# ExcitingSystems/exciting-environments

Measured on AMD Instinct MI355X. Metric: env-steps/sec + achieved HBM GB/s, PMSM Euler fp32 batch=2^22, 1/2/4/8 GPU, higher is better.
Workload: dtype f32

## Files before the change

### exciting-environments_amd/csrc/excenv_api.hip

```cpp
#include <algorithm>
#include <cstdarg>
#include <cstdio>
#include <dlfcn.h>
#include "launch.hpp"

static_assert(EXCENV_FAULT == 0, "EXCENV_FAULT builds exist for tools/isa_guards_selftest.sh only (single objects, never linked into the library)");

namespace excenv {

static thread_local char g_err[512] = "";
thread_local const char* g_last_launch = "";

void set_error(const char* fmt, ...) {
  va_list ap;
  va_start(ap, fmt);
  vsnprintf(g_err, sizeof(g_err), fmt, ap);
  va_end(ap);
}

int launch_transpose(int dtype, int64_t M, int64_t N, const void* in, void* out, hipStream_t stream);
int launch_param_sum(int dtype, int64_t B, int n, const void* const* per_env, void* out, void* workspace, hipStream_t stream);

EnvVTable vtable_pendulum();
EnvVTable vtable_msd();
// ... 6 lines not shown
static const EnvVTable* table(int env) {
  static const EnvVTable T[EXCENV_NUM_ENVS + 1] = {vtable_pendulum(), vtable_msd(),  vtable_cartpole(), vtable_acrobot(),
                                                   vtable_tank(),     vtable_pmsm(), vtable_pmsm_sat()};
  if (env < 0 || env > EXCENV_NUM_ENVS) return nullptr;
  return &T[env];
}

static const EnvVTable* table_public(int env) { return (env >= 0 && env < EXCENV_NUM_ENVS) ? table(env) : nullptr; }

static const EnvVTable* table_for(int env, const excenv_props_t* props, int* rc) {
  *rc = EXCENV_OK;
  if (env < 0 || env >= EXCENV_NUM_ENVS) return nullptr;
  if (props && props->pmsm_lut) {
    const excenv_pmsm_lut_t* l = props->pmsm_lut;
    if (env != EXCENV_PMSM) { set_error("pmsm_lut is only valid for EXCENV_PMSM"); *rc = EXCENV_EINVAL; return nullptr; }
    if (l->n_d < 2 || l->n_q < 2 || !l->grid_d || !l->grid_q || !l->tables) {
      set_error("pmsm_lut: need n_d, n_q >= 2 and non-NULL grid / table pointers");
      *rc = EXCENV_EINVAL;
      return nullptr;
    }
    return table(EXCENV_NUM_ENVS);
  }
  return table(env);
}

static const excenv_launch_opts_t kDefaultOpts = {0, 0, 0, 0};

static int check_opts(const char* fn, const excenv_launch_opts_t*& o) {
  if (!o) o = &kDefaultOpts;
  const int v = o->envs_per_lane;
  if (!(v == 0 || v == 1 || v == 2 || v == 4)) { set_error("%s: opts.envs_per_lane must be 0, 1, 2 or 4 (got %d)", fn, v); return EXCENV_EINVAL; }
  if (o->env_major_mode < 0 || o->env_major_mode > 3) { set_error("%s: opts.env_major_mode must be 0, 1, 2 or 3", fn); return EXCENV_EINVAL; }
  if (o->lds_pad_bytes < 0 || o->lds_pad_bytes > 150 * 1024) { set_error("%s: opts.lds_pad_bytes out of range", fn); return EXCENV_EINVAL; }
  if ((o->flags & ~(EXCENV_OPT_NO_FUSED_ACTIONS | EXCENV_OPT_KEEP_CONSTANT_COLUMNS)) != 0) { set_error("%s: opts.flags has unknown bits set (0x%x)", fn, (unsigned)o->flags); return EXCENV_EINVAL; }
  return EXCENV_OK;
}

static int check_common(const char* fn, int env, int solver, int dtype, int64_t B) {
  if (env < 0 || env >= EXCENV_NUM_ENVS) { set_error("%s: bad env id %d", fn, env); return EXCENV_EINVAL; }
  if (solver < 0 || solver >= EXCENV_NUM_SOLVERS) { set_error("%s: bad solver id %d", fn, solver); return EXCENV_EINVAL; }
  if (dtype != EXCENV_F32 && dtype != EXCENV_F64) { set_error("%s: bad dtype id %d", fn, dtype); return EXCENV_EINVAL; }
  if (B < 0 || B > ((int64_t)1 << 31) * BLOCK) { set_error("%s: bad batch size %lld", fn, (long long)B); return EXCENV_EINVAL; }
  return EXCENV_OK;
}

static int check_control(const char* fn, int env, const excenv_control_t*& c) {
  if (c && c->n_control == 0) c = nullptr;
  if (!c) return EXCENV_OK;
  if (c->n_control < 0 || c->n_control > EXCENV_MAX_CONTROL) { set_error("%s: bad n_control %d", fn, c->n_control); return EXCENV_EINVAL; }
  for (int j = 0; j < c->n_control; ++j) {
    if (c->control_idx[j] < 0 || c->control_idx[j] >= table_public(env)->S) { set_error("%s: control_idx[%d] out of range", fn, j); return EXCENV_EINVAL; }
    if (!c->reference[j]) { set_error("%s: reference[%d] is NULL", fn, j); return EXCENV_ENULL; }
  }
  return EXCENV_OK;
}

}

using namespace excenv;

extern "C" {

int excenv_abi_version(void) { return EXCENV_ABI_VERSION; }

const char* excenv_last_error(void) { return g_err; }

const char* excenv_last_launch(void) { return g_last_launch; }
// ... 689 lines not shown
```

### exciting-environments_amd/csrc/kernels.hpp

```cpp
#pragma once
#include "rk.hpp"
#include "sim_clock.hpp"
#include "sim_plan.hpp"

namespace excenv {

#ifndef EXCENV_FAULT
#define EXCENV_FAULT 0
#endif
template <typename T, class M> struct KProps {
  static constexpr int N = M::P + 2 * M::S + 2 * M::A;
  T scalar[N];
  const T* ptr[N];
  const T* lut_gd;
  const T* lut_gq;
  const T* lut_tab;
  int32_t lut_nd, lut_nq;
  int32_t lut_lds;
};

template <typename T, class M> struct StepArgs {
  KProps<T, M> kp;
  int64_t B;
  const T* state_in[M::S];
// ... 359 lines not shown
      gym_outputs<M, T>(st[0], ob, c, ka.n_control, ka.control_idx, rref, ka.reward + i, ka.terminated + i,
                        ka.truncated + i * tw, 1);
    }
  }
}

template <typename T, int V> constexpr bool aem_shape_ok() { return V * (int)sizeof(T) == 16; }
#define EXCENV_INLINE_ASM_M0_PUSH _Pragma("clang diagnostic push") _Pragma("clang diagnostic ignored \"-Winline-asm\"")
#if EXCENV_FAULT & 4
#define EXCENV_LDS_DIRECT_LOAD(SRC, M0V) EXCENV_INLINE_ASM_M0_PUSH                                                               \
  asm volatile("s_mov_b32 m0, %1\n\tglobal_load_lds_dwordx4 %0, off" ::"v"(SRC), "s"(M0V) : "memory", "m0");                 \
  _Pragma("clang diagnostic pop")
#else
#define EXCENV_LDS_DIRECT_LOAD(SRC, M0V) EXCENV_INLINE_ASM_M0_PUSH                                                               \
  asm volatile("s_mov_b32 m0, %1\n\ts_nop 0\n\tglobal_load_lds_dwordx4 %0, off" ::"v"(SRC), "s"(M0V) : "memory", "m0");      \
  _Pragma("clang diagnostic pop")
#endif
constexpr int AEM_BLOCK_BYTES = 1024 + 16;
template <class M> constexpr int aem_np() { return M::ID == EXCENV_ACROBOT ? 2 : 4; }
template <class M, typename T, int V> constexpr size_t aem_lds_bytes() { return (size_t)(BLOCK / 64) * V * aem_np<M>() * AEM_BLOCK_BYTES; }

template <class M, typename T, bool GENERAL, bool AEM, bool LGYM, int STATES, int SOLVER = -1, bool PLAIN_AHEAD = false, int V = 0> constexpr int sim_min_waves() {
  if (LGYM && (M::ID == EXCENV_ACROBOT || M::ID == EXCENV_CART_POLE) && sizeof(T) == 4 && SOLVER == EXCENV_EULER) return 3;
  if (LGYM && M::ID == EXCENV_ACROBOT && sizeof(T) == 4) return 2;
  if (GENERAL && M::ID == EXCENV_PENDULUM && sizeof(T) == 8) return 2;
  if (AEM && M::IS_PMSM && !M::HAS_LUT && sizeof(T) == 8 && STATES == 0) return 2;
  if (V == 2 && PLAIN_AHEAD && !GENERAL && !AEM && !LGYM && M::IS_PMSM && !M::HAS_LUT && sizeof(T) == 8 && STATES == 0 && SOLVER == EXCENV_EULER) return 2;
  return 1;
}
#define EXCENV_SIM_KERNEL_ATTR __attribute__((amdgpu_waves_per_eu(sim_min_waves<M, T, GENERAL, AEM, LGYM, STATES, SOLVER, AHEAD, V>())))
template <class M, typename T, int SOLVER, bool AHEAD, bool GENERAL, int V, int STATES, bool LUT_LDS = false, bool AEM = false, bool LGYM = false,
          int NT = BLOCK>
__global__ void __launch_bounds__(NT) EXCENV_SIM_KERNEL_ATTR sim_ahead_kernel(const SimArgs<T, M> ka) {
  constexpr bool ACC_T = false;
  [[maybe_unused]] constexpr T acc_step = T(0), acc_end = T(0);
#include "sim_ahead_body.inc"
}
template <class M, typename T, int SOLVER, bool GENERAL, int V, int STATES, bool LUT_LDS = false, int NT = BLOCK>
__global__ void __launch_bounds__(NT) __attribute__((amdgpu_waves_per_eu(sim_min_waves<M, T, GENERAL, false, false, STATES, SOLVER>())))
sim_ahead_acc_t_kernel(const SimArgs<T, M> ka, const T acc_step, const T acc_end) {
  constexpr bool AHEAD = true, AEM = false, LGYM = false, ACC_T = true;
#include "sim_ahead_body.inc"
}

template <typename T, class M> struct ControlFillArgs {
  KProps<T, M> kp;
  int64_t B, rows;
  int32_t n_control, tiled;
  int32_t control_idx[EXCENV_MAX_CONTROL];
  const T* reference[EXCENV_MAX_CONTROL];
  T* obs;
  int64_t o_sk, o_sc, tile_pitch;
};

template <class M, typename T, int V> __global__ void __launch_bounds__(BLOCK) control_fill_kernel(const ControlFillArgs<T, M> ka) {
  const int64_t b0 = ((int64_t)blockIdx.x * BLOCK + threadIdx.x) * V;
  if (b0 >= ka.B) return;
  T* base = ka.obs + (ka.tiled ? (b0 / EXCENV_TILE) * ka.tile_pitch + (b0 % EXCENV_TILE) : b0);
#pragma unroll
  for (int j = 0; j < EXCENV_MAX_CONTROL; ++j) {
    if (j < ka.n_control) {
      const int f = ka.control_idx[j];
      const T lo = ka.kp.scalar[M::P + f], hi = ka.kp.scalar[M::P + M::S + f];
      T r[V], c[V];
      load_v<T, V>(ka.reference[j] + b0, r);
#pragma unroll
      for (int v = 0; v < V; ++v) c[v] = normalize(r[v], lo, hi);
      T* col = base + (M::O + j) * ka.o_sc;
      for (int64_t n = blockIdx.y; n < ka.rows; n += gridDim.y) store_stream<T, V>(col + n * ka.o_sk, c);
    }
  }
}

template <typename T, class M> struct TrajGymArgs {
// ... 147 lines not shown
```

### exciting-environments_amd/csrc/launch.hpp

```cpp
#pragma once
#include <cstdint>
#include <cstdio>
#include <cstring>
#include <type_traits>
#include "kernels_emr.hpp"
#include "refgen.hpp"
#include "rew_vjp.hpp"
#include "step_jac.hpp"
#include "step_vjp.hpp"
#include "vjp.hpp"

namespace excenv {

void set_error(const char* fmt, ...);
static thread_local bool g_attr_failed = false;
extern thread_local const char* g_last_launch;

struct StepCall {
  int vec_pref;
  int solver, dtype;
  int64_t B;
  const excenv_props_t* props;
  const excenv_control_t* control;
  double tau;
// ... 273 lines not shown
  const bool general = batched || ka.n_control > 0 || ka.reward != nullptr;
  int V = 1;
  if (!general) {
    bool ok = true;
    for (int j = 0; j < M::S; ++j) ok &= aligned16(ka.state_in[j]) && aligned16(ka.state_out[j]);
    int want = sc.vec_pref > 0 ? sc.vec_pref : 1;
    if (want > VMAX) want = VMAX;
    while (want > 1 && (sc.B % want) != 0) want >>= 1;
    if (ok) V = want;
  }
  const int64_t lanes = sc.B / V;
  const dim3 grid((unsigned)((lanes + BLOCK - 1) / BLOCK)), block(BLOCK);
  constexpr int VWs = 16 / (int)sizeof(T);
  const bool dense = !general && V == 1 && (M::O % VWs) == 0 && (M::O / VWs) > 1;
  const size_t step_lds = lut_lds_bytes<T, M>(ka.kp, 0, dense ? sizeof(T) * BLOCK * M::O : 0);
  with_solver(sc.solver, [&](auto solver) {
    constexpr int SOLVER = decltype(solver)::value;
    if (general) launch_dyn(&step_kernel<M, T, SOLVER, true, 1>, grid, block, step_lds, sc.stream, ka);
    else with_const<1, 2, 4>(V, [&](auto v) {
      constexpr int VV = decltype(v)::value;
      if constexpr (VV <= VMAX) launch_dyn(&step_kernel<M, T, SOLVER, false, VV>, grid, block, step_lds, sc.stream, ka);
      return true;
    });
    return true;
  });
  g_last_launch = general ? "step_kernel (general)" : V == 1 ? "step_kernel (V=1)" : V == 2 ? "step_kernel (V=2)" : "step_kernel (V=4)";
  return check_launch("excenv_step");
}

template <class M, typename T, int SOLVER, int SEM>
static bool launch_lane_major(const SimPlan& p, SimArgs<T, M> ka, size_t lds_pad, T acc_step, T acc_end, hipStream_t stream) {
  constexpr bool ACC_T = SEM == EXCENV_SEM_AHEAD_ACCUMULATED_T;
  const size_t lds = lut_lds_bytes<T, M>(ka.kp, lds_pad);
  return with_const<SIM_GENERAL, SIM_LEAN, SIM_LEAN_GYM, SIM_AEM>(p.form, [&](auto form) {
    return with_const<1, 2, 4>(p.V, [&](auto v) {
      return with_const<BLOCK, WIDE_THREADS>(p.threads, [&](auto nt) {
        constexpr SimForm F = (SimForm)decltype(form)::value;
        constexpr int V = decltype(v)::value, NT = decltype(nt)::value;
        constexpr bool GEN = F == SIM_GENERAL;
        if constexpr (!sim_instantiated(SimPlan{F, false, V, NT, 0, 0, false, 0, ACC_T}, SEM, M::ID, M::A, (int)sizeof(T), SOLVER,
                                        M::HAS_LUT)) {
          return false;
        } else {
          const dim3 grid((unsigned)((ka.B / V + NT - 1) / NT)), block(NT);
          const size_t l = F == SIM_AEM ? aem_lds_bytes<M, T, V>() + lds : lds;
          with_flag(GEN ? ka.truncated != nullptr : ka.straj[0] != nullptr, [&](auto st) {
            return with_flag(ka.kp.lut_lds != 0, [&](auto lut_lds) {
              constexpr int STATES = (GEN ? -2 : 0) + decltype(st)::value;
              constexpr bool LUT_LDS = M::HAS_LUT && decltype(lut_lds)::value;
              if constexpr (ACC_T)
                launch_dyn(&sim_ahead_acc_t_kernel<M, T, SOLVER, GEN, V, STATES, LUT_LDS, NT>, grid, block, l, stream, ka, acc_step, acc_end);
              else
                launch_dyn(&sim_ahead_kernel<M, T, SOLVER, SEM == EXCENV_SEM_AHEAD, GEN, V, STATES, LUT_LDS, F == SIM_AEM, F == SIM_LEAN_GYM, NT>,
                           grid, block, l, stream, ka);
              return true;
            });
          });
          return true;
        }
      });
    });
  });
}

template <class M, typename T, int SOLVER, int SEM>
static bool launch_em(const SimPlan& p, const SimArgs<T, M>& ka, hipStream_t stream) {
// ... 107 lines not shown
  const bool emr = p.form == SIM_EMR, env_major = emr || p.form == SIM_EM || p.form == SIM_EM_GENERAL;
  if (emr) ka.a_wg = p.period;
  if (!env_major) {
    ka.row_sync = p.row_sync;
    ka.keep_const = (sc.keep_const && sc.traj_layout == EXCENV_LAYOUT_LANE_MAJOR && ka.o_sb == 1 && ka.s_sb == 1) ? 1 : 0;
    const int64_t wg_envs = (int64_t)p.threads * p.V;
    auto wg_off = [&](int layout, int64_t sb, int64_t per_tile) -> int64_t {
      if (layout == EXCENV_LAYOUT_TILED) return (wg_envs == TILE) ? per_tile : -1;
      return wg_envs * sb;
    };
    ka.a_wg = wg_off(sc.action_layout, ka.a_sb, sc.K * M::A * TILE);
    ka.o_wg = wg_off(sc.traj_layout, ka.o_sb, (N + 1) * OW * TILE);
    ka.s_wg = wg_off(sc.traj_layout, ka.s_sb, (N + 1) * TILE);
    if (ka.a_wg < 0 || ka.o_wg < 0 || ka.s_wg < 0) {
      set_error("excenv_sim_ahead: tiled layout needs unbatched properties, no gym trajectories, 16-byte aligned buffers and the %d-byte dtype (control columns are filled by a second launch)", 4);
      return EXCENV_EUNSUPPORTED;
    }
  }
  const size_t lds_pad = (size_t)sc.lds_pad + p.row_lds;
  const T acc_step = (T)(sc.obs_stepsize * (double)sc.substeps), acc_end = (T)((sc.obs_stepsize * (double)sc.substeps) * (double)sc.K);
  auto launch = [&](auto solver, auto sem) {
    constexpr int SOLVER = decltype(solver)::value, SEM = decltype(sem)::value;
    if (emr) return launch_emr<M, T, SOLVER, SEM>(p, ka, sc.stream);
    if (env_major) return launch_em<M, T, SOLVER, SEM>(p, ka, sc.stream);
    return launch_lane_major<M, T, SOLVER, SEM>(p, ka, lds_pad, acc_step, acc_end, sc.stream);
  };
  if (!sim_instantiated(p, sc.semantics, M::ID, M::A, (int)sizeof(T), sc.solver, M::HAS_LUT) || !with_solver(sc.solver, [&](auto solver) {
        return with_const<EXCENV_SEM_STEP, EXCENV_SEM_AHEAD, EXCENV_SEM_AHEAD_ACCUMULATED_T>(sc.semantics, [&](auto sem) { return launch(solver, sem); });
      })) {
    set_error("excenv_sim_ahead: no kernel instantiation for plan '%s' (semantics %d, %d-byte elements)", plan_name(p), sc.semantics,
              (int)sizeof(T));
    return EXCENV_EINVAL;
  }
  g_last_launch = plan_name(p);
  if (int rc = check_launch(emr ? "excenv_sim_ahead (env-major fused, register ring)" : env_major ? "excenv_sim_ahead (env-major fused)" : "excenv_sim_ahead"))
    return rc;
  if (p.split_control) {
    ControlFillArgs<T, M> fa;
    std::memset(&fa, 0, sizeof(fa));
    fa.kp = ka.kp;
    fa.B = sc.B;
    fa.rows = N + 1;
    fa.n_control = ka.n_control;
    fa.tiled = tiled_t ? 1 : 0;
    for (int j = 0; j < ka.n_control; ++j) {
      fa.control_idx[j] = ka.control_idx[j];
      fa.reference[j] = ka.reference[j];
    }
    fa.obs = ka.obs;
    fa.o_sk = ka.o_sk;
    fa.o_sc = ka.o_sc;
    fa.tile_pitch = (N + 1) * OW * TILE;
    bool v4 = (sizeof(T) == 4) && (sc.B % 4 == 0) && aligned16(ka.obs);
    for (int j = 0; j < ka.n_control; ++j) v4 &= aligned16(fa.reference[j]);
    const int64_t lanes = v4 ? sc.B / 4 : sc.B;
    const dim3 fgrid((unsigned)((lanes + BLOCK - 1) / BLOCK), (unsigned)((N + 1 < 64) ? N + 1 : 64)), fblock(BLOCK);
    if (v4) {
      if constexpr (sizeof(T) == 4) hipLaunchKernelGGL((control_fill_kernel<M, T, 4>), fgrid, fblock, 0, sc.stream, fa);
    } else {
      hipLaunchKernelGGL((control_fill_kernel<M, T, 1>), fgrid, fblock, 0, sc.stream, fa);
    }
    return check_launch("excenv_sim_ahead (control columns)");
  }
  return EXCENV_OK;
}

template <class M, typename T> static int launch_traj_gym(const TrajGymCall& gc) {
// ... 151 lines not shown
```

### exciting-environments_amd/csrc/sim_ahead_body.inc

```
  static_assert(!ACC_T || (AHEAD && !AEM && !LGYM), "accumulated time: AHEAD structure, no row-major action windows, no lean gym outputs");
  constexpr int S = M::S, A = M::A, O = M::O;
  extern __shared__ __align__(16) unsigned char excenv_smem[];
  static_assert(NT == BLOCK || (!GENERAL && !AEM && !M::HAS_LUT), "wide workgroups: lean instantiations only (plain or with gym outputs)");
  constexpr bool ROW_BARRIER = NT > BLOCK;
  static_assert(!(GENERAL && V > 1), "per-environment property sets: one environment per lane");
  static_assert(GENERAL == (STATES < 0), "STATES -1 / -2 (general, with / without the gym outputs' code) and 0 / 1 (lean)");
  static_assert(!LGYM || (!GENERAL && !M::HAS_LUT && aem_shape_ok<T, V>()), "lean gym outputs: widest lean form, no look-up model");
  constexpr int NC = GENERAL ? V : 1;
  constexpr bool GYM = GENERAL && STATES == -1;
  static_assert(!AEM || (!GENERAL && !M::HAS_LUT && aem_shape_ok<T, V>() && (16 / (int)sizeof(T)) % A == 0),
                "row-major actions are fused into the widest lean instantiation only");
  const int64_t blk0 = (int64_t)blockIdx.x * (NT * V);
  const unsigned lane_env = threadIdx.x * V;
  const int64_t i0 = blk0 + lane_env;
  Ctx<T, M> cs[NC];
#pragma unroll
  for (int v = 0; v < NC; ++v) {
    load_ctx<GENERAL>(cs[v], ka.kp, (i0 + v < ka.B) ? i0 + v : 0, ka.dt, ka.env_tau, ka.adv_coef);
    cs[v].lin_stop = ka.lin_stop;
    cs[v].lin_div = T(ka.K - 1);
    cs[v].lin_last = ka.K - 1;
  }
  Ctx<T, M>& c = cs[0];
#define EXCENV_CX(v) cs[GENERAL ? (v) : 0]
  stage_lut<M, T>(c, ka.kp);
  if constexpr (M::HAS_LUT) c.lut_lds = LUT_LDS ? 1 : 0;
  if (i0 >= ka.B) return;

  T st[V][S];
#pragma unroll
  for (int j = 0; j < S; ++j) {
    T tmp[V];
    load_v<T, V>(ka.state_in[j] + blk0 + lane_env, tmp);
// ... 125 lines not shown
  constexpr int KC_OBS = 2, KC_LEAF = 6;
  bool keep = false;
  if constexpr (KEEPC) {
    if (__builtin_expect(ka.keep_const != 0, 1)) {
      T kept_o[V], kept_s[V];
      load_v<T, V>(o_blk + KC_OBS * ka.o_sc + o_lane, kept_o);
      if (with_states) load_v<T, V>(ka.straj[KC_LEAF] + s_blk + s_lane, kept_s);
      bool same = true;
#pragma unroll
      for (int v = 0; v < V; ++v) {
        T sv0[S], ob0[O];
#pragma unroll
        for (int j = 0; j < S; ++j) sv0[j] = st[v][j];
        if constexpr (AHEAD) M::post(sv0, c);
        M::observe(sv0, c, ob0);
        same = same & same_bits(kept_o[v], ob0[KC_OBS]);
        if (with_states) same = same & same_bits(kept_s[v], sv0[KC_LEAF]);
      }
      keep = __builtin_amdgcn_readfirstlane((int)(__builtin_amdgcn_ballot_w64(!same) == 0)) != 0;
      if constexpr (V == 1 && !ROW_BARRIER) {
        if (ka.row_sync == 2) {
          unsigned* vote = reinterpret_cast<unsigned*>(excenv_smem);
          if (threadIdx.x == 0) *vote = 0u;
          __syncthreads();
          if (!keep && (threadIdx.x & 63u) == 0u) *vote = 1u;
          __syncthreads();
          keep = __builtin_amdgcn_readfirstlane(*vote) == 0u;
          __syncthreads();
        }
      }
    }
  }

  auto save_row = [&](int64_t n, T (&sv)[V][S]) {
#pragma unroll
    for (int v = 0; v < V; ++v) {
#pragma unroll
      for (int j = 0; j < S; ++j) sv[v][j] = st[v][j];
      if constexpr (AHEAD) {
        if constexpr (M::HAS_LUT) M::post_q(sv[v], c, memo[v]);
        else M::post(sv[v], EXCENV_CX(v));
        if constexpr (M::IS_PMSM) {
          if (deadtime_on) {
            sv[v][0] = aux[v].prev_clip[0];
            sv[v][1] = aux[v].prev_clip[1];
          } else {
            sv[v][0] = T(0);
            sv[v][1] = T(0);
          }
        }
      }
    }
    T ob[V][O];
#pragma unroll
    for (int v = 0; v < V; ++v) M::observe(sv[v], EXCENV_CX(v), ob[v]);
    T* orow = o_blk + n * ka.o_sk;
    bool direct = true;
    if constexpr (ROW_BARRIER) {
      __builtin_amdgcn_s_barrier();
    } else if constexpr (V == 1 && !M::HAS_LUT && !AEM) {
      if (ka.row_sync == 2) {
        constexpr int VE = 16 / (int)sizeof(T), CH = NT / (64 * VE), NW = NT / 64;
        const int OWr = O + (GENERAL ? ka.n_control : 0);
        const int NS = OWr + (with_states ? S : 0);
        T* buf = reinterpret_cast<T*>(excenv_smem) + (unsigned)(n & 1) * (unsigned)(NS * NT);
#pragma unroll
// ... 120 lines not shown
      }
      if (n > 0) {
        store_stream<T, V>(ka.reward + (n - 1) * ka.g_sk + e0, rew);
        store_flags<V>(ka.terminated + (n - 1) * ka.g_sk + e0, fl);
      }
    }
    if constexpr (LGYM && M::IS_PMSM) {
      T rew[V];
      uint8_t fl[V];
#pragma unroll
      for (int v = 0; v < V; ++v) {
        rew[v] = pmsm_reward<M, T>(sv[v], c, has_id, g_id[v], has_iq, g_iq[v], has_tq, g_tq[v]);
        const T nd = normalize(sv[v][3], c.smin[3], c.smax[3]), nq = normalize(sv[v][4], c.smin[4], c.smax[4]);
        fl[v] = sqrt_exceeds_one(nd * nd + nq * nq);
      }
      const int64_t e0 = blk0 + lane_env;
      store_flags<V>(ka.truncated + n * ka.t_sk + e0, fl);
      if (n > 0) {
        store_stream<T, V>(ka.reward + (n - 1) * ka.g_sk + e0, rew);
        store_flags<V>(ka.terminated + (n - 1) * ka.g_sk + e0, fl);
      }
    }
    if constexpr (GYM) {
      if (ka.truncated != nullptr) {
        const int64_t e = i0;
        uint8_t* tr = ka.truncated + e * ka.t_sb + n * ka.t_sk;
        const bool tail = n > 0;
        T* rw = tail ? ka.reward + e * ka.g_sb + (n - 1) * ka.g_sk : nullptr;
        uint8_t* te = tail ? ka.terminated + e * ka.g_sb + (n - 1) * ka.g_sk : nullptr;
        gym_outputs<M, T>(sv[0], ob[0], c, ka.n_control, ka.control_idx, rref[0], rw, te, tr, ka.t_sc);
      }
    }
  };
  auto publish_last = [&](const T (&sv)[V][S]) {
#pragma unroll
    for (int j = 0; j < S; ++j) {
      T tmp[V];
#pragma unroll
      for (int v = 0; v < V; ++v) tmp[v] = sv[v][j];
      store_v<T, V>(ka.last_state[j] + blk0 + lane_env, tmp);
    }
  };
  T sv[V][S];
  if (N == 0) {
    save_row(0, sv);
    publish_last(sv);
    return;
  }

  T a0[A][V], a1[A][V];
  int64_t k = 0, kn = 0;
  int32_t sub = 0, subn = 0;
  constexpr int VW = 16 / (int)sizeof(T);
  constexpr int SP = AEM ? VW / A : 1;
  constexpr int NP = aem_np<M>();
  constexpr int EPI = 64 / NP;
  static_assert(64 % NP == 0, "a load instruction covers whole windows");
  const unsigned wave = threadIdx.x / 64u, lane64 = threadIdx.x % 64u;
  const unsigned wave_off = AEM ? __builtin_amdgcn_readfirstlane(wave * (unsigned)(V * NP * AEM_BLOCK_BYTES)) : 0u;
  const unsigned wave_lds = (unsigned)(uintptr_t)(__attribute__((address_space(3))) unsigned char*)excenv_smem + wave_off;
  const unsigned rd_lane = (lane64 / EPI) * AEM_BLOCK_BYTES + (lane64 % EPI) * (NP * 16u);
  const unsigned ld_piece = lane64 % NP;
  const uint64_t ld_lane_off = AEM ? ((uint64_t)(wave * 64u + lane64 / NP) * V) * (uint64_t)ka.a_sb : 0;
  const int32_t n_pieces = AEM ? (int32_t)((ka.K * A) / VW) : 0;
  constexpr int NSTORE = O + ((STATES != 0) ? S : 0);
  const bool aem_aligned = AEM && ((n_pieces * V) % NP) == 0;
  unsigned aem_ph[V];
  int32_t w_hi[V];
#pragma unroll
  for (int v = 0; v < V; ++v) {
    aem_ph[v] = aem_aligned ? (unsigned)((((uintptr_t)a_blk >> 4) + (uint64_t)v * (uint64_t)(uint32_t)n_pieces) % NP) : 0u;
    w_hi[v] = -1;
  }
  auto dma_window = [&](int v, int32_t w) __attribute__((always_inline)) {
    if constexpr (AEM) {
      int32_t pc = w * NP + (int32_t)ld_piece - (int32_t)aem_ph[v];
      pc = pc < 0 ? 0 : (pc < n_pieces ? pc : n_pieces - 1);
      const T* lane_src = a_blk + ld_lane_off + (int64_t)pc * VW;
// ... 85 lines not shown
    subn = sub + 1;
    if (subn == ka.substeps) { subn = 0; kn = k + 1; }
  };
  const int64_t klast = ka.K - 1;
  auto next_row = [&]() __attribute__((always_inline)) -> int64_t {
    if constexpr (ACC_T) {
      kn = __builtin_amdgcn_readfirstlane(clk.row_next());
      dt_step = clk.step_size();
      clk.advance();
      return kn;
    } else {
      next_index();
      return (kn < klast) ? kn : klast;
    }
  };
  if constexpr (AEM) {
#pragma unroll
    for (int v = 0; v < V; ++v) {
      dma_window(v, 0);
      w_hi[v] = 0;
    }
    asm volatile("s_waitcnt vmcnt(0)" ::: "memory");
  }
  load_action(0, a0);
  if constexpr (AEM) {
    asm volatile("s_waitcnt vmcnt(0)" ::: "memory");
    fill_pending = false;
  }
  constexpr bool PINGPONG = SOLVER == EXCENV_EULER && !M::HAS_LUT;
  if constexpr (PINGPONG) {
    for (int64_t n = 0;; n += 2) {
      int64_t k1 = next_row();
      load_action(k1, a1);
      save_row(n, sv);
      if (n == N) break;
      advance(a0, a1, k, k1);
      k = kn;
      sub = subn;
      k1 = next_row();
      load_action(k1, a0);
      save_row(n + 1, sv);
      if (n + 1 == N) break;
      advance(a1, a0, k, k1);
      k = kn;
      sub = subn;
    }
  } else {
    for (int64_t n = 0;; ++n) {
      const int64_t k1 = next_row();
      load_action(k1, a1);
      save_row(n, sv);
      if (n == N) break;
      advance(a0, a1, k, k1);
#pragma unroll
      for (int q = 0; q < A; ++q)
#pragma unroll
        for (int v = 0; v < V; ++v) a0[q][v] = a1[q][v];
      k = kn;
      sub = subn;
    }
  }
  publish_last(sv);
#undef EXCENV_CX
```

### exciting-environments_amd/csrc/sim_plan.hpp

```cpp
#pragma once
#include <cstddef>
#include <cstdint>
#include "../../include/excenv.h"

namespace excenv {

constexpr int BLOCK = 256;
constexpr int EM_LANES = 64;
static_assert(EXCENV_TILE % BLOCK == 0, "a workgroup must not straddle tiles of the tiled layout");
constexpr int EM_TK = 8;
constexpr int EMR_MAX_RING_REGS = 128;

constexpr int auto_envs_per_lane(int64_t B, int vmax) {
  while (vmax > 1 && (B / vmax) < (int64_t)1024 * 64 * (vmax >= 4 ? 2 : 1)) vmax >>= 1;
  return vmax;
}
constexpr bool widest_form_pays(int64_t B, int vmax) { return (B / vmax) >= (int64_t)1024 * 64; }

constexpr int64_t ROW_SYNC_MIN_BATCH = (int64_t)1 << 17;
constexpr int WIDE_THREADS = 1024;
constexpr int64_t WIDE_MIN_WORKGROUPS = 256;
constexpr bool sim_wide_ok(int env, int elem, int solver, bool lut) {
  return solver == EXCENV_EULER && !lut &&
         (env == EXCENV_PENDULUM || env == EXCENV_MASS_SPRING_DAMPER || (env == EXCENV_FLUID_TANK && elem == 4));
}
constexpr bool sim_wide_gym_ok(int env, int elem, int solver, bool lut) {
  return sim_wide_ok(env, elem, solver, lut) && (env != EXCENV_PENDULUM || elem == 4);
}
constexpr bool aem_fits(int A, int elem) { return (16 / elem) % A == 0; }
constexpr int em_tk(int elem) { return elem == 4 ? EM_TK : EM_TK / 2; }
constexpr size_t em_lds_elems(int elem, int S, int O) { return (size_t)EM_LANES * (128 / elem + 16 / elem + S * (em_tk(elem) + 1) + O); }
constexpr bool emr_supported(bool lut) { return !lut; }
constexpr int emr_const_leaf(bool pmsm) { return pmsm ? 6 : -1; }
constexpr int emr_derived_leaf(bool pmsm, bool ahead) { return (pmsm && ahead) ? 5 : -1; }
constexpr int emr_ring_leaves(int S, bool pmsm, bool ahead) {
  return S - (emr_const_leaf(pmsm) >= 0 ? 1 : 0) - (emr_derived_leaf(pmsm, ahead) >= 0 ? 1 : 0);
}
constexpr int emr_rows(int S, bool pmsm, bool ahead, int elem) {
  return (emr_ring_leaves(S, pmsm, ahead) * 32 <= EMR_MAX_RING_REGS / (elem / 4) ? 128 : 64) / elem;
}
constexpr int64_t emr_period(int64_t K, int64_t W) {
  int64_t g = W, y = (K + 1) % W;
  while (y) { const int64_t t = g % y; g = y; y = t; }
  return W / g;
}
constexpr int64_t align_up(int64_t x) { return (x + 255) & ~(int64_t)255; }
constexpr int64_t sim_workspace_bytes(int S, int A, int O, int elem, int64_t B, int64_t K, int32_t substeps, int32_t n_control,
                                      int action_layout, int traj_layout, bool with_state_traj) {
  const int64_t rows = K * substeps + 1;
  return (action_layout == EXCENV_LAYOUT_ENV_MAJOR ? align_up(elem * K * A * B) : 0) +
         (traj_layout == EXCENV_LAYOUT_ENV_MAJOR ? align_up(elem * rows * (O + n_control) * B) +
                                                       (with_state_traj ? S * align_up(elem * rows * B) : 0) : 0);
}
inline int align_of(const void* p) { const uintptr_t a = reinterpret_cast<uintptr_t>(p) | 128u; return (int)(a & (~a + 1)); }
struct SimFacts {
  int env, S, A, O, elem, solver, semantics;
  int64_t B, K;
  int32_t substeps; int action_layout, traj_layout;
  bool per_env_props, lut;
  int n_control; bool refs_given, gym, state_traj;
  int al_actions, al_obs, al_state_io, al_straj;
  int al_reward, al_terminated, al_truncated, al_refs;
  int envs_per_lane, env_major_mode, flags;
  bool workspace; int al_workspace; int64_t workspace_bytes;
};
enum SimForm { SIM_GENERAL, SIM_LEAN, SIM_LEAN_GYM, SIM_AEM, SIM_EM, SIM_EM_GENERAL, SIM_EMR };
struct SimPlan {
  SimForm form;
  bool via_workspace;
  int V, threads;
  int row_sync, row_lds;
  bool split_control;
  int64_t period;
  bool acc_t = false;
};
constexpr bool sim_instantiated(const SimPlan& p, int semantics, int env, int A, int elem, int solver, bool lut) {
  const bool acc_t = semantics == EXCENV_SEM_AHEAD_ACCUMULATED_T;
  if ((elem != 4 && elem != 8) || solver < 0 || solver >= EXCENV_NUM_SOLVERS || semantics < EXCENV_SEM_STEP ||
      semantics > EXCENV_SEM_AHEAD_ACCUMULATED_T || p.acc_t != acc_t)
    return false;
  const int VA = 16 / elem;
  switch (p.form) {
    case SIM_GENERAL: return p.V == 1 && p.threads == BLOCK;
    case SIM_LEAN:
      if (p.threads == WIDE_THREADS) return p.V == VA && sim_wide_ok(env, elem, solver, lut);
      return p.threads == BLOCK && (p.V == 1 || p.V == 2 || (p.V == 4 && elem == 4));
    case SIM_LEAN_GYM:
      return !acc_t && !lut && p.V == VA && (p.threads == BLOCK || (p.threads == WIDE_THREADS && sim_wide_gym_ok(env, elem, solver, lut)));
    case SIM_AEM: return !acc_t && !lut && aem_fits(A, elem) && p.V == VA && p.threads == BLOCK;
    case SIM_EM:
    case SIM_EM_GENERAL: return !acc_t && p.V == 1 && p.threads == EM_LANES;
    case SIM_EMR: return !acc_t && emr_supported(lut) && p.V == 1 && p.threads == EM_LANES;
  }
  return false;
}

namespace plan_detail {
constexpr int vmax(const SimFacts& f) { return 16 / f.elem; }
constexpr bool acc_t(const SimFacts& f) { return f.semantics == EXCENV_SEM_AHEAD_ACCUMULATED_T; }
constexpr bool takes_widest(const SimFacts& f) {
  int want = f.envs_per_lane > 0 ? f.envs_per_lane : (widest_form_pays(f.B, vmax(f)) ? vmax(f) : 1);
  if (f.envs_per_lane == 0 && f.env == EXCENV_ACROBOT && f.solver != EXCENV_EULER && want > 2) want = 2;
  return want == vmax(f);
}
constexpr bool reads_row_major_actions(const SimFacts& f) {
  const int vm = vmax(f);
  if ((f.flags & EXCENV_OPT_NO_FUSED_ACTIONS) || acc_t(f) || f.lut || f.per_env_props || f.gym || !f.refs_given || f.al_obs < 16) return false;
  if (f.action_layout != EXCENV_LAYOUT_ENV_MAJOR || f.traj_layout != EXCENV_LAYOUT_LANE_MAJOR) return false;
  if (f.K < 1 || !aem_fits(f.A, f.elem) || (f.K * f.A) % vm != 0) return false;
  if ((f.B % (64 * vm)) != 0) return false;
  if (f.al_actions < 16) return false;
  if ((int64_t)BLOCK * vm * f.K * f.A >= ((int64_t)1 << 32)) return false;
  return takes_widest(f);
}
// ... 29 lines not shown
  const bool aem_candidate = reads_row_major_actions(f) && states16;
  const bool split = !f.per_env_props && (!f.gym || lean_gym) && f.n_control > 0 && !em_t && (!em_a || aem_candidate) && f.refs_given;
  const bool general = f.per_env_props || (f.n_control > 0 && !split) || (f.gym && !lean_gym);
  const bool aem = aem_candidate && !general;
  SimPlan p{general ? SIM_GENERAL : lean_gym ? SIM_LEAN_GYM : aem ? SIM_AEM : SIM_LEAN, false, 1, BLOCK, 0, 0, split, 0};
  const bool vec_ok = !general && states16 && (!em_a || aem) && !em_t && f.al_actions >= 16 && f.al_obs >= 16;
  if (vec_ok) {
    int want = f.envs_per_lane > 0 ? f.envs_per_lane : ((aem || lean_gym) ? VMAX : auto_envs_per_lane(f.B, VMAX));
    if (f.envs_per_lane == 0) {
      if (f.env == EXCENV_ACROBOT && f.solver != EXCENV_EULER && want > 2) want = 2;
      if (f.lut && want > (f.solver == EXCENV_EULER ? 2 : 1)) want = f.solver == EXCENV_EULER ? 2 : 1;
      if (f.env == EXCENV_PMSM && !f.lut && f.elem == 4 && !f.state_traj && !aem && !lean_gym &&
          want > (f.solver == EXCENV_EULER ? 1 : 2))
        want = f.solver == EXCENV_EULER ? 1 : 2;
      if (f.elem == 4 && !aem && !lean_gym && want > 2 &&
          ((f.env == EXCENV_CART_POLE && f.solver != EXCENV_EULER) || (f.env == EXCENV_PENDULUM && f.solver == EXCENV_TSIT5)))
        want = 2;
    }
    if (want > VMAX) want = VMAX;
    while (want > 1 && (f.B % want) != 0) want >>= 1;
    p.V = want;
  }
  if (tiled) {
    constexpr int VT = EXCENV_TILE / BLOCK;
    p.V = (VT > VMAX || !vec_ok) ? 1 : VT;
  }
  const int row_bytes = 2 * (f.O + f.n_control + (f.state_traj ? f.S : 0)) * BLOCK * f.elem;
  if (p.V == 1 && !f.gym && lm_t && f.B >= ROW_SYNC_MIN_BATCH)
    p.row_sync = (!f.lut && (f.B % BLOCK) == 0 && f.al_obs >= 16 && f.al_straj >= 16 && row_bytes <= (64 << 10)) ? 2 : 1;
  if (p.row_sync == 2) p.row_lds = row_bytes;
  if (sim_wide_ok(f.env, f.elem, f.solver, f.lut) && (!lean_gym || sim_wide_gym_ok(f.env, f.elem, f.solver, f.lut)) &&
      (p.form == SIM_LEAN || p.form == SIM_LEAN_GYM) && !tiled && p.V == VMAX && f.B / p.V >= WIDE_THREADS * WIDE_MIN_WORKGROUPS)
    p.threads = WIDE_THREADS;
  return p;
}
}

constexpr SimPlan sim_plan(const SimFacts& f) {
  using namespace plan_detail;
  if (fused_env_major(f)) return plan_env_major(f);
  const bool em_a = f.action_layout == EXCENV_LAYOUT_ENV_MAJOR, em_t = f.traj_layout == EXCENV_LAYOUT_ENV_MAJOR;
  const int64_t need = sim_workspace_bytes(f.S, f.A, f.O, f.elem, f.B, f.K, f.substeps, f.n_control, f.action_layout,
                                           f.traj_layout, f.state_traj);
  if (!reads_row_major_actions(f) && !f.gym && f.workspace && need > 0 && f.workspace_bytes >= need && f.B > 0 && (em_a || em_t)) {
    SimFacts w = f;
    if (em_a) { w.action_layout = EXCENV_LAYOUT_LANE_MAJOR; w.al_actions = f.al_workspace; }
    if (em_t) { w.traj_layout = EXCENV_LAYOUT_LANE_MAJOR; w.al_obs = f.al_workspace; w.al_straj = f.state_traj ? f.al_workspace : 128; }
    w.flags = 0;
    SimPlan p = plan_lane_major(w);
    p.via_workspace = true;
    p.acc_t = acc_t(f);
    return p;
  }
  SimPlan p = plan_lane_major(f);
  p.acc_t = acc_t(f);
  return p;
}
constexpr const char* plan_name(const SimPlan& p) {
  const bool wide = p.threads == WIDE_THREADS;
  if (p.acc_t) {
    if (p.via_workspace) return "transposition workspace + sim_ahead_kernel (accumulated t)";
    if (p.form == SIM_GENERAL) return "sim_ahead_kernel (general, accumulated t)";
    if (p.V == 1) return "sim_ahead_kernel (V=1, accumulated t)";
    if (p.V == 2) return wide ? "sim_ahead_kernel (V=2, 1024 threads, accumulated t)" : "sim_ahead_kernel (V=2, accumulated t)";
    return wide ? "sim_ahead_kernel (V=4, 1024 threads, accumulated t)" : "sim_ahead_kernel (V=4, accumulated t)";
  }
  if (p.via_workspace) return "transposition workspace + sim_ahead_kernel";
  switch (p.form) {
    case SIM_GENERAL: return "sim_ahead_kernel (general)";
    case SIM_LEAN_GYM: return wide ? "sim_ahead_kernel (lean, gym outputs, 1024 threads)" : "sim_ahead_kernel (lean, gym outputs)";
    case SIM_AEM: return "sim_ahead_kernel (row-major actions fused)";
    case SIM_EM: return "sim_ahead_em_kernel";
    case SIM_EM_GENERAL: return "sim_ahead_em_kernel (general)";
    case SIM_EMR: return "sim_ahead_emr_kernel";
    case SIM_LEAN: break;
  }
  if (p.V == 1) return "sim_ahead_kernel (V=1)";
  if (p.V == 2) return wide ? "sim_ahead_kernel (V=2, 1024 threads)" : "sim_ahead_kernel (V=2)";
  return wide ? "sim_ahead_kernel (V=4, 1024 threads)" : "sim_ahead_kernel (V=4)";
}

}
```

### exciting-environments_amd/exciting_environments_amd/_native.py

```python
from __future__ import annotations

import ctypes
import os
from typing import Optional, Sequence

import torch

MAX_STATE, MAX_ACTION, MAX_STATIC, MAX_CONTROL = 8, 2, 9, 8
LAYOUT_ENV_MAJOR, LAYOUT_LANE_MAJOR, LAYOUT_TILED = 0, 1, 2
TILE = 1024
SEM_STEP, SEM_AHEAD = 0, 1
SEM_AHEAD_ACCUMULATED_T = 2
SEMANTICS = {"step": SEM_STEP, "ahead": SEM_AHEAD, "ahead_accumulated_t": SEM_AHEAD_ACCUMULATED_T}
F32, F64 = 0, 1
JAC_STATE, JAC_OBS = 0, 1
JAC_ROWS = {"state": JAC_STATE, "obs": JAC_OBS}
OPT_NO_FUSED_ACTIONS = 1
OPT_KEEP_CONSTANT_COLUMNS = 2
ABI_VERSION = 7

_LIB_PATH = os.environ.get(
    "EXCENV_HIP_LIB", os.path.join(os.path.dirname(os.path.abspath(__file__)), "lib", "libexcenv_hip.so"))


class Param(ctypes.Structure):
    _fields_ = [("value", ctypes.c_double), ("per_env", ctypes.c_void_p)]


class PmsmLut(ctypes.Structure):
    _fields_ = [("n_d", ctypes.c_int32), ("n_q", ctypes.c_int32), ("grid_d", ctypes.c_void_p),
                ("grid_q", ctypes.c_void_p), ("tables", ctypes.c_void_p)]


class Props(ctypes.Structure):
    _fields_ = [
        ("static_params", Param * MAX_STATIC),
        ("state_min", Param * MAX_STATE),
        ("state_max", Param * MAX_STATE),
        ("action_min", Param * MAX_ACTION),
        ("action_max", Param * MAX_ACTION),
        ("pmsm_lut", ctypes.POINTER(PmsmLut)),
    ]


class LaunchOpts(ctypes.Structure):

    _fields_ = [("envs_per_lane", ctypes.c_int32), ("env_major_mode", ctypes.c_int32), ("lds_pad_bytes", ctypes.c_int32),
                ("flags", ctypes.c_int32)]


class TrajGym(ctypes.Structure):
# ... 438 lines not shown
```

### include/excenv.h

```cpp
#ifndef EXCENV_H
#define EXCENV_H

#include <stdint.h>

#ifdef __cplusplus
extern "C" {
#endif

#define EXCENV_ABI_VERSION 7

typedef enum {
  EXCENV_PENDULUM = 0,
  EXCENV_MASS_SPRING_DAMPER = 1,
  EXCENV_CART_POLE = 2,
  EXCENV_ACROBOT = 3,
  EXCENV_FLUID_TANK = 4,
  EXCENV_PMSM = 5,
  EXCENV_NUM_ENVS = 6
} excenv_env_t;

typedef enum { EXCENV_EULER = 0, EXCENV_RK4 = 1, EXCENV_TSIT5 = 2, EXCENV_NUM_SOLVERS = 3 } excenv_solver_t;

typedef enum { EXCENV_F32 = 0, EXCENV_F64 = 1 } excenv_dtype_t;

// ... 7 lines not shown
#define EXCENV_MAX_STATIC 9
#define EXCENV_MAX_CONTROL 8

typedef struct {
  double value;
  const void* per_env;
} excenv_param_t;

typedef struct {
  int32_t n_d, n_q;
  const void* grid_d;
  const void* grid_q;
  const void* tables;
} excenv_pmsm_lut_t;

typedef struct {
  excenv_param_t static_params[EXCENV_MAX_STATIC];
  excenv_param_t state_min[EXCENV_MAX_STATE];
  excenv_param_t state_max[EXCENV_MAX_STATE];
  excenv_param_t action_min[EXCENV_MAX_ACTION];
  excenv_param_t action_max[EXCENV_MAX_ACTION];
  const excenv_pmsm_lut_t* pmsm_lut;
} excenv_props_t;

typedef struct {
  int32_t n_control;
  int32_t control_idx[EXCENV_MAX_CONTROL];
  const void* reference[EXCENV_MAX_CONTROL];
  const void* obs_reference[EXCENV_MAX_CONTROL];
} excenv_control_t;

#define EXCENV_OPT_NO_FUSED_ACTIONS 1
#define EXCENV_OPT_KEEP_CONSTANT_COLUMNS 2
typedef struct {
  int32_t envs_per_lane;
  int32_t env_major_mode;
  int32_t lds_pad_bytes;
  int32_t flags;
} excenv_launch_opts_t;

typedef struct {
  void* reward;
  uint8_t* terminated;
  uint8_t* truncated;
} excenv_traj_gym_t;

int excenv_abi_version(void);
const char* excenv_last_error(void);
const char* excenv_last_launch(void);
int excenv_env_dims(int env, int32_t* S, int32_t* A, int32_t* O, int32_t* P);
int64_t excenv_step_bytes(int env, int dtype);
int64_t excenv_sim_ahead_bytes(int env, int dtype, int with_state_traj);

int excenv_step(int env, int solver, int dtype, int64_t B,
                const excenv_props_t* props, const excenv_control_t* control, double tau,
                const void* const* state_in, const void* action,
                void* const* state_out, void* obs, const excenv_launch_opts_t* opts, void* stream);

int32_t excenv_truncated_width(int env, int32_t n_control);
int excenv_gym_step(int env, int solver, int dtype, int64_t B,
                    const excenv_props_t* props, const excenv_control_t* control, double tau,
                    const void* const* state_in, const void* action,
                    void* const* state_out, void* obs, void* reward, uint8_t* terminated, uint8_t* truncated,
                    const excenv_launch_opts_t* opts, void* stream);

int excenv_sim_ahead(int env, int solver, int dtype, int64_t B, int64_t K, int32_t substeps,
// ... 107 lines not shown
```

Baseline: 95.38 billion.

## Stage PMSM Euler fp32 trajectory rows through LDS before streaming stores

Adds a dedicated sim_ahead_staged_kernel for the PMSM Euler fp32 path with four environments per lane. It computes observation and state rows two environments at a time, writes them into a per-wave LDS slice, then reads them back as full V=4 vectors for streaming global stores. The aim is to cut live registers and give wider store transactions on the trajectory write path. The cost is extra LDS traffic and shared memory per block. The path is auto-selected when the heuristic picks four envs per lane, and opt-in/opt-out flags are added.

```diff
diff --git a/exciting-environments_amd/csrc/excenv_api.hip b/exciting-environments_amd/csrc/excenv_api.hip
--- a/exciting-environments_amd/csrc/excenv_api.hip
+++ b/exciting-environments_amd/csrc/excenv_api.hip
@@ -62,7 +62,7 @@
   if (!(v == 0 || v == 1 || v == 2 || v == 4)) { set_error("%s: opts.envs_per_lane must be 0, 1, 2 or 4 (got %d)", fn, v); return EXCENV_EINVAL; }
   if (o->env_major_mode < 0 || o->env_major_mode > 3) { set_error("%s: opts.env_major_mode must be 0, 1, 2 or 3", fn); return EXCENV_EINVAL; }
   if (o->lds_pad_bytes < 0 || o->lds_pad_bytes > 150 * 1024) { set_error("%s: opts.lds_pad_bytes out of range", fn); return EXCENV_EINVAL; }
-  if ((o->flags & ~(EXCENV_OPT_NO_FUSED_ACTIONS | EXCENV_OPT_KEEP_CONSTANT_COLUMNS)) != 0) { set_error("%s: opts.flags has unknown bits set (0x%x)", fn, (unsigned)o->flags); return EXCENV_EINVAL; }
+  if ((o->flags & ~(EXCENV_OPT_NO_FUSED_ACTIONS | EXCENV_OPT_KEEP_CONSTANT_COLUMNS | EXCENV_OPT_STAGED_ROWS | EXCENV_OPT_NO_STAGED_ROWS)) != 0) { set_error("%s: opts.flags has unknown bits set (0x%x)", fn, (unsigned)o->flags); return EXCENV_EINVAL; }
   return EXCENV_OK;
 }
 
diff --git a/exciting-environments_amd/csrc/kernels.hpp b/exciting-environments_amd/csrc/kernels.hpp
--- a/exciting-environments_amd/csrc/kernels.hpp
+++ b/exciting-environments_amd/csrc/kernels.hpp
@@ -415,14 +415,20 @@
 template <class M, typename T, int SOLVER, bool AHEAD, bool GENERAL, int V, int STATES, bool LUT_LDS = false, bool AEM = false, bool LGYM = false,
           int NT = BLOCK>
 __global__ void __launch_bounds__(NT) EXCENV_SIM_KERNEL_ATTR sim_ahead_kernel(const SimArgs<T, M> ka) {
-  constexpr bool ACC_T = false;
+  constexpr bool ACC_T = false, STAGED = false;
   [[maybe_unused]] constexpr T acc_step = T(0), acc_end = T(0);
 #include "sim_ahead_body.inc"
 }
 template <class M, typename T, int SOLVER, bool GENERAL, int V, int STATES, bool LUT_LDS = false, int NT = BLOCK>
 __global__ void __launch_bounds__(NT) __attribute__((amdgpu_waves_per_eu(sim_min_waves<M, T, GENERAL, false, false, STATES, SOLVER>())))
 sim_ahead_acc_t_kernel(const SimArgs<T, M> ka, const T acc_step, const T acc_end) {
-  constexpr bool AHEAD = true, AEM = false, LGYM = false, ACC_T = true;
+  constexpr bool AHEAD = true, AEM = false, LGYM = false, ACC_T = true, STAGED = false;
+#include "sim_ahead_body.inc"
+}
+template <class M, typename T, int SOLVER> __global__ void __launch_bounds__(BLOCK) __attribute__((amdgpu_waves_per_eu(1))) sim_ahead_staged_kernel(const SimArgs<T, M> ka) {
+  constexpr bool AHEAD = true, GENERAL = false, LUT_LDS = false, AEM = false, LGYM = false, ACC_T = false, STAGED = true;
+  constexpr int V = 4, STATES = 1, NT = BLOCK;
+  [[maybe_unused]] constexpr T acc_step = T(0), acc_end = T(0);
 #include "sim_ahead_body.inc"
 }
 
diff --git a/exciting-environments_amd/csrc/launch.hpp b/exciting-environments_amd/csrc/launch.hpp
--- a/exciting-environments_amd/csrc/launch.hpp
+++ b/exciting-environments_amd/csrc/launch.hpp
@@ -329,6 +329,16 @@
 static bool launch_lane_major(const SimPlan& p, SimArgs<T, M> ka, size_t lds_pad, T acc_step, T acc_end, hipStream_t stream) {
   constexpr bool ACC_T = SEM == EXCENV_SEM_AHEAD_ACCUMULATED_T;
   const size_t lds = lut_lds_bytes<T, M>(ka.kp, lds_pad);
+  if (p.staged) {
+    if constexpr (staged_rows_ok(M::ID, (int)sizeof(T), SOLVER, M::HAS_LUT, SEM)) {
+      if (ka.straj[0] == nullptr || (ka.B % (BLOCK * STAGED_ENVS_PER_LANE)) != 0) return false;
+      launch_dyn(&sim_ahead_staged_kernel<M, T, SOLVER>, dim3((unsigned)(ka.B / (BLOCK * STAGED_ENVS_PER_LANE))), dim3(BLOCK),
+                 staged_lds_bytes(M::S, M::O) + lds, stream, ka);
+      return true;
+    } else {
+      return false;
+    }
+  }
   return with_const<SIM_GENERAL, SIM_LEAN, SIM_LEAN_GYM, SIM_AEM>(p.form, [&](auto form) {
     return with_const<1, 2, 4>(p.V, [&](auto v) {
       return with_const<BLOCK, WIDE_THREADS>(p.threads, [&](auto nt) {
@@ -502,7 +512,7 @@
               (int)sizeof(T));
     return EXCENV_EINVAL;
   }
-  g_last_launch = plan_name(p);
+  g_last_launch = launch_name(p);
   if (int rc = check_launch(emr ? "excenv_sim_ahead (env-major fused, register ring)" : env_major ? "excenv_sim_ahead (env-major fused)" : "excenv_sim_ahead"))
     return rc;
   if (p.split_control) {
diff --git a/exciting-environments_amd/csrc/sim_ahead_body.inc b/exciting-environments_amd/csrc/sim_ahead_body.inc
--- a/exciting-environments_amd/csrc/sim_ahead_body.inc
+++ b/exciting-environments_amd/csrc/sim_ahead_body.inc
@@ -1,4 +1,7 @@
   static_assert(!ACC_T || (AHEAD && !AEM && !LGYM), "accumulated time: AHEAD structure, no row-major action windows, no lean gym outputs");
+  static_assert(!STAGED || (M::IS_PMSM && !M::HAS_LUT && sizeof(T) == 4 && SOLVER == EXCENV_EULER && AHEAD && !GENERAL && V == 4 &&
+                             STATES == 1 && !AEM && !LGYM && !ACC_T && NT == BLOCK),
+                "rows staged in LDS: the PMSM Euler fp32 instantiation with four environments per lane and state trajectories only");
   constexpr int S = M::S, A = M::A, O = M::O;
   extern __shared__ __align__(16) unsigned char excenv_smem[];
   static_assert(NT == BLOCK || (!GENERAL && !AEM && !M::HAS_LUT), "wide workgroups: lean instantiations only (plain or with gym outputs)");
@@ -190,6 +193,67 @@
     }
   }
 
+  constexpr int STG_NS = STAGED ? (O - 1) + (S - 1) : 0;
+  [[maybe_unused]] unsigned stg_off = 0;
+  if constexpr (STAGED) stg_off = __builtin_amdgcn_readfirstlane((threadIdx.x >> 6) * (unsigned)(STG_NS * 64 * V)) + (threadIdx.x & 63u) * V;
+  [[maybe_unused]] auto save_row_staged = [&](int64_t n) __attribute__((always_inline)) {
+    if constexpr (STAGED) {
+      T* slice = reinterpret_cast<T*>(excenv_smem) + stg_off;
+      T kob[V], kst[V];
+#pragma unroll
+      for (int v = 0; v < V; ++v) asm volatile("" : "+v"(st[v][KC_LEAF]));
+#pragma unroll
+      for (int p = 0; p < V; p += 2) {
+        T svp[2][S], obp[2][O];
+#pragma unroll
+        for (int u = 0; u < 2; ++u) {
+#pragma unroll
+          for (int j = 0; j < S; ++j) svp[u][j] = st[p + u][j];
+          M::post(svp[u], c);
+          svp[u][0] = deadtime_on ? aux[p + u].prev_clip[0] : T(0);
+          svp[u][1] = deadtime_on ? aux[p + u].prev_clip[1] : T(0);
+          M::observe(svp[u], c, obp[u]);
+          kob[p + u] = obp[u][KC_OBS];
+          kst[p + u] = svp[u][KC_LEAF];
+        }
+#pragma unroll
+        for (int q = 0; q < O; ++q) {
+          if (q == KC_OBS) continue;
+          const T two[2] = {obp[0][q], obp[1][q]};
+          store_v<T, 2>(slice + (q - (q > KC_OBS)) * (64 * V) + p, two);
+        }
+#pragma unroll
+        for (int j = 0; j < S; ++j) {
+          if (j == KC_LEAF) continue;
+          const T two[2] = {svp[0][j], svp[1][j]};
+          store_v<T, 2>(slice + ((O - 1) + j - (j > KC_LEAF)) * (64 * V) + p, two);
+        }
+        __builtin_amdgcn_sched_barrier(0);
+      }
+      T* orow = o_blk + n * ka.o_sk;
+#pragma unroll
+      for (int q = 0; q < O; ++q) {
+        if (q == KC_OBS) {
+          if (!keep) store_stream<T, V>(orow + q * ka.o_sc + o_lane, kob);
+          continue;
+        }
+        T tmp[V];
+        load_v<T, V>(slice + (q - (q > KC_OBS)) * (64 * V), tmp);
+        store_stream<T, V>(orow + q * ka.o_sc + o_lane, tmp);
+      }
+#pragma unroll
+      for (int j = 0; j < S; ++j) {
+        T* dst = ka.straj[j] + s_blk + n * ka.s_sk + s_lane;
+        if (j == KC_LEAF) {
+          if (!keep) store_stream<T, V>(dst, kst);
+          continue;
+        }
+        T tmp[V];
+        load_v<T, V>(slice + ((O - 1) + j - (j > KC_LEAF)) * (64 * V), tmp);
+        store_stream<T, V>(dst, tmp);
+      }
+    }
+  };
   auto save_row = [&](int64_t n, T (&sv)[V][S]) {
 #pragma unroll
     for (int v = 0; v < V; ++v) {
@@ -376,7 +440,17 @@
       }
     }
   };
-  auto publish_last = [&](const T (&sv)[V][S]) {
+  auto publish_last = [&](T (&sv)[V][S]) {
+    if constexpr (STAGED) {
+#pragma unroll
+      for (int v = 0; v < V; ++v) {
+#pragma unroll
+        for (int j = 0; j < S; ++j) sv[v][j] = st[v][j];
+        M::post(sv[v], c);
+        sv[v][0] = deadtime_on ? aux[v].prev_clip[0] : T(0);
+        sv[v][1] = deadtime_on ? aux[v].prev_clip[1] : T(0);
+      }
+    }
 #pragma unroll
     for (int j = 0; j < S; ++j) {
       T tmp[V];
@@ -385,9 +459,10 @@
       store_v<T, V>(ka.last_state[j] + blk0 + lane_env, tmp);
     }
   };
+#define EXCENV_SAVE_ROW(n) do { if constexpr (STAGED) save_row_staged(n); else save_row(n, sv); } while (0)
   T sv[V][S];
   if (N == 0) {
-    save_row(0, sv);
+    EXCENV_SAVE_ROW(0);
     publish_last(sv);
     return;
   }
@@ -539,14 +614,14 @@
     for (int64_t n = 0;; n += 2) {
       int64_t k1 = next_row();
       load_action(k1, a1);
-      save_row(n, sv);
+      EXCENV_SAVE_ROW(n);
       if (n == N) break;
       advance(a0, a1, k, k1);
       k = kn;
       sub = subn;
       k1 = next_row();
       load_action(k1, a0);
-      save_row(n + 1, sv);
+      EXCENV_SAVE_ROW(n + 1);
       if (n + 1 == N) break;
       advance(a1, a0, k, k1);
       k = kn;
@@ -556,7 +631,7 @@
     for (int64_t n = 0;; ++n) {
       const int64_t k1 = next_row();
       load_action(k1, a1);
-      save_row(n, sv);
+      EXCENV_SAVE_ROW(n);
       if (n == N) break;
       advance(a0, a1, k, k1);
 #pragma unroll
@@ -568,4 +643,5 @@
     }
   }
   publish_last(sv);
+#undef EXCENV_SAVE_ROW
 #undef EXCENV_CX
diff --git a/exciting-environments_amd/csrc/sim_plan.hpp b/exciting-environments_amd/csrc/sim_plan.hpp
--- a/exciting-environments_amd/csrc/sim_plan.hpp
+++ b/exciting-environments_amd/csrc/sim_plan.hpp
@@ -44,6 +44,11 @@
   while (y) { const int64_t t = g % y; g = y; y = t; }
   return W / g;
 }
+constexpr bool staged_rows_ok(int env, int elem, int solver, bool lut, int semantics) {
+  return env == EXCENV_PMSM && elem == 4 && solver == EXCENV_EULER && !lut && semantics == EXCENV_SEM_AHEAD;
+}
+constexpr int STAGED_ENVS_PER_LANE = 4;
+constexpr size_t staged_lds_bytes(int S, int O) { return (size_t)(BLOCK / 64) * (size_t)(S + O - 2) * 64 * 16; }
 constexpr int64_t align_up(int64_t x) { return (x + 255) & ~(int64_t)255; }
 constexpr int64_t sim_workspace_bytes(int S, int A, int O, int elem, int64_t B, int64_t K, int32_t substeps, int32_t n_control,
                                       int action_layout, int traj_layout, bool with_state_traj) {
@@ -73,6 +78,7 @@
   bool split_control;
   int64_t period;
   bool acc_t = false;
+  bool staged = false;
 };
 constexpr bool sim_instantiated(const SimPlan& p, int semantics, int env, int A, int elem, int solver, bool lut) {
   const bool acc_t = semantics == EXCENV_SEM_AHEAD_ACCUMULATED_T;
@@ -80,6 +86,8 @@
       semantics > EXCENV_SEM_AHEAD_ACCUMULATED_T || p.acc_t != acc_t)
     return false;
   const int VA = 16 / elem;
+  if (p.staged)
+    return p.form == SIM_LEAN && p.V == STAGED_ENVS_PER_LANE && p.threads == BLOCK && staged_rows_ok(env, elem, solver, lut, semantics);
   switch (p.form) {
     case SIM_GENERAL: return p.V == 1 && p.threads == BLOCK;
     case SIM_LEAN:
@@ -175,6 +183,10 @@
   if (sim_wide_ok(f.env, f.elem, f.solver, f.lut) && (!lean_gym || sim_wide_gym_ok(f.env, f.elem, f.solver, f.lut)) &&
       (p.form == SIM_LEAN || p.form == SIM_LEAN_GYM) && !tiled && p.V == VMAX && f.B / p.V >= WIDE_THREADS * WIDE_MIN_WORKGROUPS)
     p.threads = WIDE_THREADS;
+  p.staged = !(f.flags & EXCENV_OPT_NO_STAGED_ROWS) &&
+             ((f.flags & EXCENV_OPT_STAGED_ROWS) || auto_envs_per_lane(f.B, VMAX) == STAGED_ENVS_PER_LANE) && p.form == SIM_LEAN && p.V == STAGED_ENVS_PER_LANE && p.threads == BLOCK &&
+             !tiled && lm_a && lm_t && f.state_traj && (f.B % (BLOCK * STAGED_ENVS_PER_LANE)) == 0 &&
+             staged_rows_ok(f.env, f.elem, f.solver, f.lut, f.semantics);
   return p;
 }
 }
@@ -189,7 +201,7 @@
     SimFacts w = f;
     if (em_a) { w.action_layout = EXCENV_LAYOUT_LANE_MAJOR; w.al_actions = f.al_workspace; }
     if (em_t) { w.traj_layout = EXCENV_LAYOUT_LANE_MAJOR; w.al_obs = f.al_workspace; w.al_straj = f.state_traj ? f.al_workspace : 128; }
-    w.flags = 0;
+    w.flags = f.flags & (EXCENV_OPT_STAGED_ROWS | EXCENV_OPT_NO_STAGED_ROWS);
     SimPlan p = plan_lane_major(w);
     p.via_workspace = true;
     p.acc_t = acc_t(f);
@@ -222,5 +234,8 @@
   if (p.V == 2) return wide ? "sim_ahead_kernel (V=2, 1024 threads)" : "sim_ahead_kernel (V=2)";
   return wide ? "sim_ahead_kernel (V=4, 1024 threads)" : "sim_ahead_kernel (V=4)";
 }
-
-}
+constexpr const char* launch_name(const SimPlan& p) {
+  return (p.staged && !p.via_workspace) ? "sim_ahead_kernel (V=4, rows staged in LDS)" : plan_name(p);
+}
+
+}
diff --git a/exciting-environments_amd/exciting_environments_amd/_native.py b/exciting-environments_amd/exciting_environments_amd/_native.py
--- a/exciting-environments_amd/exciting_environments_amd/_native.py
+++ b/exciting-environments_amd/exciting_environments_amd/_native.py
@@ -17,6 +17,8 @@
 JAC_ROWS = {"state": JAC_STATE, "obs": JAC_OBS}
 OPT_NO_FUSED_ACTIONS = 1
 OPT_KEEP_CONSTANT_COLUMNS = 2
+OPT_STAGED_ROWS = 8
+OPT_NO_STAGED_ROWS = 16
 ABI_VERSION = 7
 
 _LIB_PATH = os.environ.get(
diff --git a/include/excenv.h b/include/excenv.h
--- a/include/excenv.h
+++ b/include/excenv.h
@@ -63,6 +63,8 @@
 
 #define EXCENV_OPT_NO_FUSED_ACTIONS 1
 #define EXCENV_OPT_KEEP_CONSTANT_COLUMNS 2
+#define EXCENV_OPT_STAGED_ROWS 8
+#define EXCENV_OPT_NO_STAGED_ROWS 16
 typedef struct {
   int32_t envs_per_lane;
   int32_t env_major_mode;
```

Result: no change. 96.18 billion (median of 6 runs) (+0.8%).
